# joshua16266261/self-play-ai

Hardware: AMD Instinct MI355X
Metric: MCTS sims/sec + self-play games/sec, Connect4 800 sims/move, 1/2/4/8 GPU (higher is better)
Workload: dtype bf16

## Files before the change

### include/spai.h

```cpp
#ifndef SPAI_H
#define SPAI_H

#include <stddef.h>
#include <stdint.h>

#ifdef __cplusplus
extern "C" {
#endif

#define SPAI_VERSION_MAJOR 0
#define SPAI_VERSION_MINOR 4

typedef enum spai_error {
    SPAI_OK = 0,
    SPAI_ERR_INVALID = -1,
    SPAI_ERR_ILLEGAL_MOVE = -2,
    SPAI_ERR_GAME_OVER = -3,
    SPAI_ERR_DEVICE = -4,
    SPAI_ERR_NAN = -5,
    SPAI_ERR_CAPACITY = -6,
    SPAI_ERR_UNSUPPORTED = -7
} spai_error;

typedef enum spai_game { SPAI_GAME_TICTACTOE = 0, SPAI_GAME_CONNECT4 = 1, SPAI_GAME_CHESS = 2 } spai_game;
// ... 72 lines not shown
                                 const float *policies , const float *values ,
                                 const int32_t *moves );
typedef struct spai_selfplay_stats {
    double sims;
    double evals;
    double games;
    double positions;
    double moves;
    double seconds;
} spai_selfplay_stats;
int spai_selfplay_run(spai_engine *eng, uint32_t n_games, uint64_t game_id_base, spai_sample_sink sink, void *user,
                      spai_selfplay_stats *stats);
int spai_selfplay_stream(spai_engine *eng, uint32_t n_games, uint32_t window, uint64_t game_id_base,
                         spai_sample_sink sink, void *user, spai_selfplay_stats *stats);

int spai_eval_cache_set_capacity(spai_engine *eng, uint64_t entries);
typedef struct spai_eval_cache_stats {
    double lookups;
    double hits;
    double inserts;
    double dropped;
    double clears;
    double capacity;
} spai_eval_cache_stats;
int spai_eval_cache_get_stats(spai_engine *eng, spai_eval_cache_stats *out);

typedef struct spai_match_player {
    int32_t eval;
    uint32_t num_searches;
    spai_net *net;
} spai_match_player;
typedef struct spai_match_config {
    uint32_t struct_size;
    uint32_t opening_plies;
    uint64_t seed;
} spai_match_config;
typedef struct spai_match_game {
    uint64_t game_id;
    int8_t a_moves_first;
    int8_t result_a;
    uint8_t n_moves;
    uint8_t moves[42];
} spai_match_game;
typedef struct spai_match_stats {
    double a_wins[2], draws[2], b_wins[2];
    double sims[2], evals[2];
    double seconds;
} spai_match_stats;
// ... 281 lines not shown
```

### self-play-ai_amd/csrc/capi.cpp

```cpp
#include <cstdarg>
#include <cstdio>
#include <cstring>
#include <new>

#include "philox.h"
#include "spai_internal.h"

namespace spai {
namespace {
thread_local char g_err[1024] = "";
}

void set_error(const char *fmt, ...) {
    va_list ap;
    va_start(ap, fmt);
    vsnprintf(g_err, sizeof(g_err), fmt, ap);
    va_end(ap);
}

namespace {
float philox_unit(uint64_t seed, uint32_t tensor, uint64_t idx) {
    uint32_t key[2] = {(uint32_t)seed, (uint32_t)(seed >> 32)};
    uint32_t ctr[4] = {(uint32_t)idx, (uint32_t)(idx >> 32), tensor, 0x5EEDu};
    uint32_t out[4];
// ... 284 lines not shown
        SPAI_PTR(values);
    }
    return net_predict(n, cnt, s, priors, values);
}

int spai_engine_set_net(spai_engine *e, spai_net *n) {
    ENG_CHECK(e);
    SPAI_CHECK(!n || n->eng == e, SPAI_ERR_INVALID, "net belongs to another engine");
    e->net = n;
    return eval_cache_clear(e);
}

int spai_eval_cache_set_capacity(spai_engine *e, uint64_t entries) {
    ENG_CHECK(e);
    return eval_cache_set_capacity(e, entries);
}

int spai_eval_cache_get_stats(spai_engine *e, spai_eval_cache_stats *out) {
    ENG_CHECK(e);
    SPAI_PTR(out);
    return eval_cache_stats(e, out);
}

int spai_trees_create(spai_engine *e, uint32_t n) { ENG_CHECK(e); return trees_create(e, n); }
int spai_tree_reset(spai_engine *e, uint32_t t, const spai_c4_state *root) { ENG_CHECK(e); return tree_reset(e, t, root); }
int spai_search(spai_engine *e, uint32_t n, const uint32_t *tree_idx, uint32_t num_searches, float *policy,
                uint32_t *child_ids, float *child_visits, uint32_t *n_children) {
    ENG_CHECK(e);
    if (n) SPAI_PTR(tree_idx);
    return search(e, n, tree_idx, num_searches, policy, child_ids, child_visits, n_children, nullptr);
}
int spai_tree_use_subtree(spai_engine *e, uint32_t t, uint32_t child) { ENG_CHECK(e); return tree_use_subtree(e, t, child); }
int spai_tree_node(spai_engine *e, uint32_t t, uint32_t node, spai_c4_state *st, uint32_t *visits, float *w) {
    ENG_CHECK(e);
    return tree_node(e, t, node, st, visits, w);
}
int spai_tree_child_stats(spai_engine *e, uint32_t t, uint32_t *child_ids, uint32_t *visits, float *value_sums,
                          float *priors, uint32_t *n_children) {
    ENG_CHECK(e);
    return tree_child_stats(e, t, child_ids, visits, value_sums, priors, n_children);
}
int spai_tree_size(spai_engine *e, uint32_t t, uint32_t *nodes) {
    ENG_CHECK(e);
    SPAI_PTR(nodes);
    return tree_size(e, t, nodes);
}
// ... 313 lines not shown
```

### self-play-ai_amd/csrc/search.hip

```cpp
#include <algorithm>
#include <cstdlib>
#include <cstring>

#include "search_internal.h"

namespace spai {
namespace {

constexpr int kLanesPerTree = 8;
constexpr int kBlock = 64;
constexpr int kTreesPerBlock = kBlock / kLanesPerTree;
constexpr uint32_t kErrNan = 1u, kErrCapacity = 2u, kErrDepth = 4u;

constexpr uint32_t kPriorMark = 0x80000000u;
constexpr int kGenShift = 49;

__device__ __forceinline__ float ucb(float sqrt_np, const uint4 &ch, float c) {
    const uint32_t n = ch.x;
    const float w = __uint_as_float(ch.y), prior = __uint_as_float(ch.z);
    const float qv = ((-w / (float)(n == 0 ? 1u : n)) + 1.0f) / 2.0f;
    const float q = n == 0 ? 0.0f : qv;
    float u = c * prior;
    u = u * sqrt_np;
    u = u / (1.0f + (float)n);
// ... 120 lines not shown
    }
    if (lane8 == 0) T.depth[t] = (uint8_t)d;
    if (status != c4::kOngoing) {
        backup_nodes(nodes, pr, d, c4::terminal_value(status), lane8);
        return kTerminal;
    }
    return kLive;
}

struct CacheBuckets {
    uint32_t b0, b1;
};
__device__ __forceinline__ CacheBuckets cache_buckets(const CacheView &C, uint64_t mine, uint64_t theirs) {
    const uint64_t h = c4::splitmix64(mine ^ (theirs * 0x9E3779B97F4A7C15ull));
    const uint32_t b0 = (uint32_t)(h >> 32) & C.mask, b1 = (uint32_t)h & C.mask;
    return CacheBuckets{b0, b1 == b0 ? (b0 ^ 1u) & C.mask : b1};
}
__device__ __forceinline__ uint4 *cache_way(const CacheView &C, uint32_t bucket, int way) {
    return C.tab + ((size_t)bucket * EvalCache::kWays + (uint32_t)way) * 4;
}

enum Claim { kClaimFull, kClaimDone, kClaimSame };
__device__ __forceinline__ Claim cache_claim(uint4 *bucket, uint32_t empty, uint64_t k0, uint64_t k1, const uint4 &e1,
                                             const uint4 &e2) {
    for (int w = empty ? __ffs(empty) - 1 : (int)EvalCache::kWays; w < (int)EvalCache::kWays; ++w) {
        uint4 *e = bucket + 4 * w;
        const unsigned long long old = atomicCAS((unsigned long long *)e, 0ull, (unsigned long long)k0);
        if (old == 0ull) {
            ((uint64_t *)e)[1] = k1;
            e[1] = e1;
            e[2] = e2;
            return kClaimDone;
        }
        if (old == k0) return kClaimSame;
    }
    return kClaimFull;
}

__device__ __forceinline__ bool cache_insert(const CacheView &C, const BatchView &B, uint32_t s, int lane8) {
    const uint64_t mine = B.mine[s], theirs = B.theirs[s];
    const uint64_t gen = (uint64_t)C.gen << kGenShift;
    const uint64_t k0 = mine | gen, k1 = theirs | gen;
    const CacheBuckets cb = cache_buckets(C, mine, theirs);
    uint4 *bk0 = cache_way(C, cb.b0, 0), *bk1 = cache_way(C, cb.b1, 0);
    const uint64_t seen0 = *(const uint64_t *)(bk0 + 4 * lane8);
    const uint64_t seen1 = *(const uint64_t *)(bk1 + 4 * lane8);
    const float4 pa = *(const float4 *)(B.priors + (size_t)s * kPriorStride);
    const float4 pb = *(const float4 *)(B.priors + (size_t)s * kPriorStride + 4);
    const float value = B.value[s];
    const uint32_t same = group_bits(__ballot(seen0 == k0 || seen1 == k0));
    const uint32_t empty0 = group_bits(__ballot(seen0 == 0ull));
    const uint32_t empty1 = cb.b1 != cb.b0 ? group_bits(__ballot(seen1 == 0ull)) : 0u;
    if (same || lane8 != 0) return false;
    const uint32_t p0 = __float_as_uint(pa.x), p2 = __float_as_uint(pa.z), p4 = __float_as_uint(pb.x),
                   p6 = __float_as_uint(pb.z);
    if (((p0 | p2 | p4 | p6) & kPriorMark) != 0u) return false;
    const uint4 e1 = make_uint4(p0 | kPriorMark, __float_as_uint(pa.y), p2 | kPriorMark, __float_as_uint(pa.w));
    const uint4 e2 = make_uint4(p4 | kPriorMark, __float_as_uint(pb.y), p6 | kPriorMark, __float_as_uint(value));
    const bool second = c4::popc32(empty1) > c4::popc32(empty0);
    Claim r = cache_claim(second ? bk1 : bk0, second ? empty1 : empty0, k0, k1, e1, e2);
    if (r == kClaimFull && cb.b1 != cb.b0) r = cache_claim(second ? bk0 : bk1, second ? empty0 : empty1, k0, k1, e1, e2);
    if (r == kClaimFull) atomicAdd(C.ctr + 1, 1u);
    return r == kClaimDone;
}
__device__ __forceinline__ void cache_count(const CacheView &C, bool claimed) {
    const uint64_t b = __ballot(claimed);
    if (b && (threadIdx.x & 63) == (uint32_t)__ffsll((unsigned long long)__ballot(true)) - 1u)
        atomicAdd(C.ctr, (uint32_t)c4::popc64(b));
}

__device__ __forceinline__ bool cache_holds(const uint4 &q0, const uint4 &q1, const uint4 &q2, uint64_t k0, uint64_t k1) {
    return (((uint64_t)q0.y << 32) | q0.x) == k0 && (((uint64_t)q0.w << 32) | q0.z) == k1 &&
           (q1.x & q1.z & q2.x & q2.z & kPriorMark) != 0u;
}

__device__ __forceinline__ void slot_leaf(const TreeView &T, const BatchView &B, const CacheView &C, uint32_t t,
                                          int lane8, uint64_t x, uint64_t o, uint8_t n) {
    const bool xm = c4::x_to_move(n);
    const uint64_t mine = xm ? x : o, theirs = xm ? o : x;
    if (lane8 == 0)
        __hip_atomic_fetch_add(T.evals + t, 1u, __ATOMIC_RELAXED, __HIP_MEMORY_SCOPE_AGENT);
    if (C.tab) {
        const CacheBuckets cb = cache_buckets(C, mine, theirs);
        const uint4 *ea = cache_way(C, cb.b0, lane8), *eb = cache_way(C, cb.b1, lane8);
// ... 1 lines not shown
        const uint64_t gen = (uint64_t)C.gen << kGenShift;
        const uint64_t k0 = mine | gen, k1 = theirs | gen;
        const bool match_a = cache_holds(a0, a1, a2, k0, k1), match_b = cache_holds(b0, b1, b2, k0, k1);
        const bool match = match_a || match_b;
        const uint4 q1 = match_a ? a1 : b1, q2 = match_a ? a2 : b2;
        const uint32_t hit = group_bits(__ballot(match));
        if (hit) {
            uint32_t slot = 0;
            if (lane8 == 0) {
                slot = B.cap - 1u - atomicAdd(B.hits, 1u);
                T.slot[t] = slot | kHitSlot;
                B.tree[slot] = t;
                B.mine[slot] = mine;
                B.theirs[slot] = theirs;
            }
            slot = (uint32_t)__shfl((int)slot, 0, kLanesPerTree);
            if (lane8 == __ffs(hit) - 1) {
                float4 *pr = (float4 *)(B.priors + (size_t)slot * kPriorStride);
                pr[0] = make_float4(__uint_as_float(q1.x & ~kPriorMark), __uint_as_float(q1.y),
                                    __uint_as_float(q1.z & ~kPriorMark), __uint_as_float(q1.w));
                pr[1] = make_float4(__uint_as_float(q2.x & ~kPriorMark), __uint_as_float(q2.y),
                                    __uint_as_float(q2.z & ~kPriorMark), 0.f);
                B.value[slot] = __uint_as_float(q2.w);
            }
            return;
        }
    }
    if (lane8 == 0) {
        const uint32_t slot = atomicAdd(B.count, 1u);
        T.slot[t] = slot;
        B.tree[slot] = t;
        B.mine[slot] = mine;
        B.theirs[slot] = theirs;
    }
}

template <bool RUN_ON>
__device__ __forceinline__ void select_tree(const TreeView &T, const BatchView &B, const CacheView &C, uint32_t t,
                                            RootInfo &root, int lane8, float c, uint32_t *err, uint32_t run_cap) {
    if (lane8 == 0) T.slot[t] = kNoSlot;
    uint64_t x, o;
    uint8_t n;
    if (!RUN_ON) {
        if (descend(T, t, root, lane8, c, err, x, o, n) == kLive) slot_leaf(T, B, C, t, lane8, x, o, n);
        return;
    }
// ... 130 lines not shown
        const bool claimed = fwd && cache_insert(C, B, s, lane8);
        cache_count(C, claimed);
    }
}

__global__ void k_root_stats(TreeView T, const uint32_t *__restrict__ active, uint32_t n_active, uint32_t *out,
                             uint32_t *max_evals) {
    const uint32_t i = blockIdx.x * blockDim.x + threadIdx.x;
    if (i >= n_active) return;
    const uint32_t t = active[i];
    atomicMax(max_evals, T.evals[t]);
    atomicAdd(max_evals + 1, T.evals[t]);
    const uint4 *nodes = T.nodes + (size_t)t * T.cap;
    const uint4 r = nodes[T.root[t]];
    out[i * 8] = r.w;
    const uint32_t nch = r.w == kNoChildren ? 0 : r.w >> 24, first = r.w & 0xFFFFFFu;
    for (uint32_t k = 0; k < 7; ++k) out[i * 8 + 1 + k] = k < nch ? nodes[first + k].x : 0u;
}

__global__ void k_trees_init(TreeView T, RootsOut R, uint32_t first_tree, uint32_t n) {
    const uint32_t i = blockIdx.x * blockDim.x + threadIdx.x;
    if (i < n) tree_clear(T, R, first_tree + i);
}
}

TreeView tree_view(spai_engine *e) {
    Trees &T = e->trees;
    return TreeView{T.nodes.p, T.cap, T.root.p, T.next_free.p, T.root_x.p, T.root_o.p, T.root_n.p, T.root_status.p,
                    T.path.p, T.depth.p, T.slot.p, T.left.p, T.evals.p};
}

static BatchView batch_view(spai_engine *e, int chain, uint32_t it, bool cached) {
    Batch &B = e->batch[chain];
    const size_t h = (size_t)(it & 1u) * B.cap;
    return BatchView{B.iter_counts.p + it, B.iter_more.p ? B.iter_more.p + it : nullptr, B.tree.p + h, B.mine.p + h, B.theirs.p + h,
                     B.priors.p + h * kPriorStride, B.value.p + h,
                     cached ? B.iter_hits.p + it : nullptr, B.cap};
}

CacheView cache_view(spai_engine *e) {
    EvalCache &C = e->cache;
    if (!C.buckets) return CacheView{nullptr, 0u, 0u, nullptr};
    return CacheView{C.table.p, C.buckets - 1u, C.gen, C.ctr.p};
}

int cache_clear(spai_engine *e) {
    EvalCache &C = e->cache;
    if (!C.buckets) return SPAI_OK;
    uint32_t fill = 0;
    SPAI_HIP(hipMemcpyAsync(&fill, C.ctr.p, 4, hipMemcpyDeviceToHost, e->stream));
    SPAI_HIP(hipStreamSynchronize(e->stream));
    C.inserts_cleared += fill;
    SPAI_HIP(hipMemsetAsync(C.table.p, 0, C.table.n * sizeof(uint4), e->stream));
    SPAI_HIP(hipMemsetAsync(C.ctr.p, 0, 4, e->stream));
    C.gen = C.gen % 32767u + 1u;
    C.fill_seen = 0;
    C.clears += 1;
    return SPAI_OK;
}

int cache_prepare(spai_engine *e, bool for_net) {
    EvalCache &C = e->cache;
    if (C.ready && C.for_net == for_net) return SPAI_OK;
    C.for_net = for_net;
    uint64_t want = 0;
    if (for_net) {
        const char *v = std::getenv("SPAI_EVAL_CACHE");
        if (C.user_set) want = C.requested;
        else if (v) want = std::strtoull(v, nullptr, 10);
        else {
            size_t free_bytes = 0, total_bytes = 0;
            SPAI_HIP(hipMemGetInfo(&free_bytes, &total_bytes));
            want = std::min<uint64_t>(EvalCache::kEntriesPerTree * std::max(1u, e->cfg.max_trees),
                                      total_bytes / EvalCache::kDefaultDeviceShare / EvalCache::kEntryBytes);
        }
    }
    uint32_t buckets = 0;
    if (want) {
        buckets = 1;
        while ((uint64_t)buckets * 2 * EvalCache::kWays <= want && buckets < (1u << 28)) buckets *= 2;
    }
    if (buckets != C.buckets) {
        SPAI_HIP(hipStreamSynchronize(e->stream));
        if (C.buckets) {
            uint32_t fill = 0;
            SPAI_HIP(hipMemcpy(&fill, C.ctr.p, 4, hipMemcpyDeviceToHost));
            C.inserts_cleared += fill;
        }
        C.buckets = 0;
        if (C.ctr.p) SPAI_HIP(hipMemsetAsync(C.ctr.p, 0, 4, e->stream));
        const bool by_default = !C.user_set && !std::getenv("SPAI_EVAL_CACHE");
        int rc = C.table.alloc((size_t)buckets * EvalCache::kWays * 4);
        while (rc != SPAI_OK && by_default) {
            (void)hipGetLastError();
            buckets = buckets / 2 >= EvalCache::kMinDefaultBuckets ? buckets / 2 : 0;
            rc = C.table.alloc((size_t)buckets * EvalCache::kWays * 4);
        }
        SPAI_TRY(rc);
        if (buckets) {
            if (!C.ctr.p) {
                SPAI_TRY(C.ctr.alloc(2));
                SPAI_HIP(hipMemsetAsync(C.ctr.p, 0, 8, e->stream));
            }
            C.buckets = buckets;
            SPAI_TRY(cache_clear(e));
        }
    }
    C.ready = true;
    return SPAI_OK;
}

constexpr double kMinChainLeaves = 64;
constexpr double kTailLeaves = 0.05;
constexpr uint32_t kTailTreeEvals = 160;
constexpr uint32_t kTailRun = 128;
static int env_int(const char *name, int dflt) {
    const char *v = std::getenv(name);
    return v ? std::atoi(v) : dflt;
}
struct ChainPolicy {
    int chains;
    uint32_t grid_cap;
};
static ChainPolicy chains_for(uint32_t n, double last_evals_per_iter) {
// ... 129 lines not shown
        SPAI_CHECK(!(root->x & root->o) && !((root->x | root->o) & ~c4::kBoard) && root->status <= c4::kWon,
                   SPAI_ERR_INVALID, "root is not a Connect4 bitboard");
        s = from_abi(*root);
    }
    T.h_root[t] = 0;
    T.h_root_state[t] = s;
    T.h_root_first[t] = 0;
    T.h_root_nch[t] = 0;
    k_trees_init<<<1, 64, 0, e->stream>>>(tree_view(e), roots_out(e), t, 1);
    SPAI_HIP(hipGetLastError());
    return upload_roots(e, t, 1);
}

static int evaluate(const Chain &c, hipStream_t st, const BatchView &bv, uint32_t grid_cap, int conc) {
    if (c.kind == SPAI_EVAL_NET)
        return net_eval_batch(c.net, st, bv.count, c.cnt, bv.mine, bv.theirs, bv.priors, bv.value, grid_cap, conc);
    k_eval_stub<<<(c.cnt + kBlock - 1) / kBlock, kBlock, 0, st>>>(bv, c.cnt, c.kind);
    return SPAI_OK;
}

int chains_launch(spai_engine *e, const uint32_t *trees, const Chain *chains, int nchain, uint32_t grid_cap, bool timed,
                  bool tail) {
    hipStream_t st = e->stream;
    uint32_t n = 0, iters = 0;
    int conc = 0;
    for (int h = 0; h < nchain; ++h) {
        const Chain &c = chains[h];
        if (!c.cnt) continue;
        n += c.cnt;
        iters = std::max(iters, c.iters);
        conc += c.kind == SPAI_EVAL_NET;
        Batch &B = e->batch[h];
        const uint32_t nc = std::max<uint32_t>(c.iters, 1) + (tail ? kTailChunk + 1 : 0);
        DevBuf<uint32_t> *ctr[3] = {&B.iter_counts, c.cache.tab ? &B.iter_hits : nullptr,
                                    tail ? &B.iter_more : nullptr};
        for (DevBuf<uint32_t> *b : ctr) {
            if (!b) continue;
            if (b->n < nc) SPAI_TRY(b->alloc(nc));
            SPAI_HIP(hipMemsetAsync(b->p, 0, (size_t)nc * 4, st));
        }
    }
    SPAI_HIP(hipMemcpyAsync(e->active.p, trees, (size_t)n * 4, hipMemcpyHostToDevice, st));
    SPAI_HIP(hipMemsetAsync(e->err.p, 0, 4, st));
    SPAI_HIP(hipMemsetAsync(e->trees.evals.p, 0, ((size_t)e->trees.n_trees + 2) * 4, st));
    if (n > chains[0].cnt) SPAI_HIP(hipEventRecord(e->ev_fork, st));
    for (int h = 1; h < nchain; ++h)
        if (chains[h].cnt) SPAI_HIP(hipStreamWaitEvent(e->chain_stream[h], e->ev_fork, 0));
    const TreeView tv = tree_view(e);
    timed = timed && e->timer.enabled;
    for (uint32_t it = 0; it < (tail ? 0u : iters); ++it) {
        for (int h = 0; h < nchain; ++h) {
            const Chain &c = chains[h];
            if (!c.cnt || it >= c.iters) continue;
            const hipStream_t sh = e->chain_stream[h];
            const BatchView bv = batch_view(e, h, it, c.cache.tab);
            const uint32_t nh = c.cnt, g8 = (nh + kTreesPerBlock - 1) / kTreesPerBlock;
            const uint32_t *act = e->active.p + c.off;
            const bool sample = timed && (it % e->timer.stride == 0);
            if (it == 0) {
                if (sample) SPAI_TRY(timer_record(e, 0, it, true, sh, h));
                k_select<false><<<g8, kBlock, 0, sh>>>(tv, bv, c.cache, act, nh, e->cfg.c, e->err.p, 0u);
                if (sample) SPAI_TRY(timer_record(e, 0, it, false, sh, h));
            }
            if (sample) SPAI_TRY(timer_record(e, 1, it, true, sh, h));
            SPAI_TRY(evaluate(c, sh, bv, grid_cap, std::max(conc, 1)));
            if (sample) SPAI_TRY(timer_record(e, 1, it, false, sh, h));
            if (it + 1 < c.iters) {
                const bool s2 = timed && ((it + 1) % e->timer.stride == 0);
                if (s2) SPAI_TRY(timer_record(e, 0, it + 1, true, sh, h));
                k_expand_select<false><<<g8, kBlock, 0, sh>>>(tv, bv, batch_view(e, h, it + 1, c.cache.tab), c.cache,
                                                              act, nh, e->cfg.c, e->err.p, 0u);
                if (s2) SPAI_TRY(timer_record(e, 0, it + 1, false, sh, h));
            } else {
                if (sample) SPAI_TRY(timer_record(e, 2, it, true, sh, h));
                k_expand<<<g8, kBlock, 0, sh>>>(tv, bv, c.cache, nh, e->err.p);
                if (sample) SPAI_TRY(timer_record(e, 2, it, false, sh, h));
            }
        }
    }
    SPAI_HIP(hipGetLastError());
    for (int h = 1; h < nchain; ++h) {
        if (!chains[h].cnt) continue;
        SPAI_HIP(hipEventRecord(e->ev_join[h], e->chain_stream[h]));
        SPAI_HIP(hipStreamWaitEvent(st, e->ev_join[h], 0));
    }
    return SPAI_OK;
}

int search_launch(spai_engine *e, uint32_t n, const uint32_t *tree_idx, uint32_t num_searches, SearchRun &R) {
    const int kind = (int)e->cfg.eval;
    hipStream_t st = e->stream;
    SPAI_TRY(cache_prepare(e, kind == SPAI_EVAL_NET));
    if (cache_nearly_full(e->cache)) SPAI_TRY(cache_clear(e));
    const char *tl_env = std::getenv("SPAI_TAIL_LEAVES");
    const char *tt_env = std::getenv("SPAI_TAIL_TREE_EVALS");
    const double tail_leaves = tl_env ? std::atof(tl_env) : kTailLeaves;
    const uint32_t tail_tree = tt_env ? (uint32_t)std::max(0, std::atoi(tt_env)) : kTailTreeEvals;
    const bool tail = num_searches > 0 && e->last_served_per_iter >= 0 &&
                      (e->last_served_per_iter < tail_leaves || e->last_max_tree_evals < tail_tree);
    const bool solved = e->last_served_per_iter == 0.0;
    const char *tr_env = std::getenv("SPAI_TAIL_RUN");
    const uint32_t tail_run =
        tr_env ? (uint32_t)std::max(1, std::atoi(tr_env)) : (solved ? std::max(num_searches, 1u) : kTailRun);
    const uint32_t tail_chunk = solved ? 1u : kTailChunk;
    const ChainPolicy pol = tail ? ChainPolicy{1, 0u} : chains_for(n, e->last_evals_per_iter);
    const int nchain = R.nchain = pol.chains;
    const CacheView cv = cache_view(e);
    for (int h = 0; h < nchain; ++h) {
        const uint32_t off = (uint32_t)((uint64_t)n * h / nchain);
        R.chain[h] = Chain{off, (uint32_t)((uint64_t)n * (h + 1) / nchain) - off, num_searches, kind, e->net, cv};
    }
    SPAI_TRY(chains_launch(e, tree_idx, R.chain, nchain, pol.grid_cap, true, tail));
    R.n_counts = num_searches;
    if (tail) {
        const TreeView tv = tree_view(e);
        const uint32_t g8 = (n + kTreesPerBlock - 1) / kTreesPerBlock;
        const uint32_t *act = e->active.p;
        k_set_left<<<(n + 255) / 256, 256, 0, st>>>(tv, act, n, num_searches);
        k_select<true><<<g8, kBlock, 0, st>>>(tv, batch_view(e, 0, 0, cv.tab), cv, act, n, e->cfg.c, e->err.p, tail_run);
        uint32_t p = 0, next = 1, more = 0, next_hits = 0;
        for (;;) {
            for (uint32_t q = 0; q < tail_chunk; ++q, ++p) {
                const BatchView bv = batch_view(e, 0, p, cv.tab);
                SPAI_TRY(evaluate(R.chain[0], st, bv, 0u, 1));
                k_expand_select<true><<<g8, kBlock, 0, st>>>(tv, bv, batch_view(e, 0, p + 1, cv.tab), cv, act, n,
                                                             e->cfg.c, e->err.p, tail_run);
            }
            SPAI_HIP(hipGetLastError());
            SPAI_HIP(hipMemcpyAsync(&next, e->batch[0].iter_counts.p + p, 4, hipMemcpyDeviceToHost, st));
            SPAI_HIP(hipMemcpyAsync(&more, e->batch[0].iter_more.p + p, 4, hipMemcpyDeviceToHost, st));
            if (cv.tab)
                SPAI_HIP(hipMemcpyAsync(&next_hits, e->batch[0].iter_hits.p + p, 4, hipMemcpyDeviceToHost, st));
            SPAI_HIP(hipStreamSynchronize(st));
            next += next_hits;
            if (next == 0 && more == 0) break;
// ... 154 lines not shown
        if (value_sums) memcpy(value_sums + k, &c.y, 4);
        if (priors) memcpy(priors + k, &c.z, 4);
    }
    return SPAI_OK;
}

int tree_size(spai_engine *e, uint32_t t, uint32_t *nodes) {
    Trees &T = e->trees;
    SPAI_CHECK(t < T.n_trees, SPAI_ERR_INVALID, "tree %u out of range", t);
    SPAI_HIP(hipMemcpy(nodes, T.next_free.p + t, 4, hipMemcpyDeviceToHost));
    return SPAI_OK;
}


int eval_cache_set_capacity(spai_engine *e, uint64_t entries) {
    e->cache.user_set = true;
    e->cache.requested = entries;
    e->cache.ready = false;
    return SPAI_OK;
}

int eval_cache_clear(spai_engine *e) { return cache_clear(e); }

int eval_cache_stats(spai_engine *e, spai_eval_cache_stats *out) {
    EvalCache &C = e->cache;
    uint32_t ctr[2] = {0, 0};
    SPAI_HIP(hipStreamSynchronize(e->stream));
    if (C.ctr.p) SPAI_HIP(hipMemcpy(ctr, C.ctr.p, 8, hipMemcpyDeviceToHost));
    out->lookups = C.lookups;
    out->hits = C.hits;
    out->inserts = C.inserts_cleared + ctr[0];
    out->dropped = ctr[1];
    out->clears = C.clears;
    out->capacity = (double)C.entries();
    return SPAI_OK;
}

}
```

### self-play-ai_amd/csrc/search_internal.h

```cpp
#pragma once
#include "spai_internal.h"

namespace spai {

struct TreeView {
    uint4 *nodes;
    uint32_t cap;
    const uint32_t *root;
    uint32_t *next_free;
    const uint64_t *root_x, *root_o;
    const uint8_t *root_n, *root_status;
    uint32_t *path;
    uint8_t *depth;
    uint32_t *slot;
    uint32_t *left;
    uint32_t *evals;
};
constexpr uint32_t kNoSlot = 0xFFFFFFFFu;
constexpr uint32_t kHitSlot = 0x80000000u;

struct BatchView {
    uint32_t *count;
    uint32_t *more;
    uint32_t *tree;
    uint64_t *mine, *theirs;
    float *priors;
    float *value;
    uint32_t *hits;
    uint32_t cap;
};

struct CacheView {
    uint4 *tab;
    uint32_t mask;
    uint32_t gen;
    uint32_t *ctr;
};

struct RootsOut {
    uint32_t *root;
    uint64_t *x, *o;
    uint8_t *n, *status;
};

constexpr int kMoveRec = 10;
constexpr int kRecRoot = 0, kRecVisits = 1, kRecPick = 8, kRecEvals = 9;
constexpr uint32_t kPickNone = 0x80000000u, kPickNoTable = 3u;
__host__ __device__ __forceinline__ uint32_t pick_word(int idx, int action, uint8_t status) {
    return (uint32_t)idx | (uint32_t)action << 8 | (uint32_t)status << 16;
}
inline int pick_index(uint32_t pick) { return (int)(pick & 0xFFu); }
inline int pick_action(uint32_t pick) { return (int)((pick >> 8) & 0xFFu); }
inline uint8_t pick_status(uint32_t pick) { return (uint8_t)((pick >> 16) & 0xFFu); }
inline uint32_t root_children(uint32_t children_word) { return children_word == kNoChildren ? 0 : children_word >> 24; }
inline const uint32_t *move_rec(const uint32_t *out, size_t i) { return out + 2 + i * kMoveRec; }

inline bool move_replays(const uint32_t *rec, const c4::State &rs, c4::State &cs) {
    const uint32_t pick = rec[kRecPick], legal = c4::legal_mask(rs.x, rs.o, rs.status);
    const int idx = pick_index(pick), a = pick_action(pick);
// ... 61 lines not shown

struct Chain {
    uint32_t off, cnt;
    uint32_t iters;
    int kind;
    spai_net *net;
    CacheView cache;
};
struct SearchRun {
    int nchain = 1;
    uint32_t n_counts = 0;
    Chain chain[spai_engine::kChains] = {};
};
constexpr uint32_t kTailChunk = 4;

TreeView tree_view(spai_engine *e);
CacheView cache_view(spai_engine *e);
inline RootsOut roots_out(spai_engine *e) {
    Trees &T = e->trees;
    return RootsOut{T.root.p, T.root_x.p, T.root_o.p, T.root_n.p, T.root_status.p};
}
int cache_prepare(spai_engine *e, bool for_net);
int cache_clear(spai_engine *e);
inline bool cache_nearly_full(const EvalCache &C) { return C.buckets && (uint64_t)C.fill_seen * 8 > C.entries() * 7; }
void cache_account(spai_engine *e, double served, double forwarded, uint32_t fill);
int check_device_errors(spai_engine *e, uint32_t err);
int chains_launch(spai_engine *e, const uint32_t *trees, const Chain *chains, int nchain, uint32_t grid_cap, bool timed,
                  bool tail);
int search_launch(spai_engine *e, uint32_t n, const uint32_t *tree_idx, uint32_t num_searches, SearchRun &R);
int search_finish(spai_engine *e, const SearchRun &R, uint32_t num_searches, const uint32_t *ch_counts, uint32_t err,
                  uint32_t max_tree_evals, double served, uint32_t cache_fill);
int move_buffers(spai_engine *e, size_t n_words);

struct Quiesce {
    spai_engine *e;
    uint32_t fresh_trees;
    ~Quiesce() {
        (void)hipStreamSynchronize(e->stream);
        for (hipStream_t cs : e->chain_stream)
            if (cs) (void)hipStreamSynchronize(cs);
        if (!fresh_trees) return;
        (void)cache_clear(e);
        (void)trees_create(e, fresh_trees);
    }
};

// ... 8 lines not shown
```

### self-play-ai_amd/csrc/spai_internal.h

```cpp
#pragma once
#include <hip/hip_runtime.h>
#include <stdint.h>

#include <string>
#include <vector>

#include "../../include/spai.h"
#include "c4.h"

namespace spai {

void set_error(const char *fmt, ...) __attribute__((format(printf, 1, 2)));

#define SPAI_HIP(expr)                                                                                  \
    do {                                                                                                \
        hipError_t e_ = (expr);                                                                         \
        if (e_ != hipSuccess) {                                                                         \
            ::spai::set_error("%s failed: %s (%s:%d)", #expr, hipGetErrorString(e_), __FILE__, __LINE__); \
            return SPAI_ERR_DEVICE;                                                                     \
        }                                                                                               \
    } while (0)

#define SPAI_CHECK(cond, code, ...)          \
    do {                                     \
// ... 72 lines not shown
    std::vector<uint32_t> h_root;
    std::vector<c4::State> h_root_state;
    std::vector<uint32_t> h_root_first;
    std::vector<uint8_t> h_root_nch;
};

struct Batch {
    uint32_t cap = 0;
    DevBuf<uint32_t> tree;
    DevBuf<uint64_t> mine, theirs;
    DevBuf<float> priors;
    DevBuf<float> value;
    DevBuf<uint32_t> iter_counts;
    DevBuf<uint32_t> iter_more;
    DevBuf<uint32_t> iter_hits;
};

struct EvalCache {
    static constexpr uint32_t kWays = 8;
    static constexpr uint64_t kEntriesPerTree = 16384;
    static constexpr uint64_t kEntryBytes = 64;
    static constexpr uint64_t kDefaultDeviceShare = 16;
    static constexpr uint32_t kMinDefaultBuckets = 1024;
    bool user_set = false;
    uint64_t requested = 0;
    bool ready = false;
    bool for_net = false;
    uint32_t buckets = 0;
    uint32_t gen = 0;
    DevBuf<uint4> table;
    DevBuf<uint32_t> ctr;
    uint32_t fill_seen = 0;
    double lookups = 0, hits = 0, inserts_cleared = 0, clears = 0;
    uint64_t entries() const { return (uint64_t)buckets * kWays; }
};

struct KernelTimer {
    bool enabled = false;
    uint32_t stride = 4;
    double total_ms[3] = {0, 0, 0};
    double launches[3] = {0, 0, 0};
    double items[3] = {0, 0, 0};
    std::vector<hipEvent_t> ev;
    size_t used = 0;
    std::vector<int> which;
    std::vector<uint32_t> iter;
    std::vector<int> chain;
};

}

struct spai_net {
    spai_engine *eng = nullptr;
    int blocks = 0, hidden = 0;
    int n_cu = 256;
    spai::DevBuf<uint16_t> w_stem, w_res, w_head, w_lin;
// ... 137 lines not shown
    void *user;
    spai_pipeline_event ev;
};
int replay_push(spai_replay *r, uint32_t n, const float *s, const float *p, const float *v,
                const Observer *obs = nullptr);
int replay_pop_now(spai_replay *r, uint32_t n, float *s, float *p, float *v);
int replay_size(spai_replay *r, uint32_t *n);
void choose_multiple(uint32_t n, uint32_t k, uint64_t seed, uint64_t stream, std::vector<uint32_t> &out);
int pipeline_run(const spai_pipeline_config *cfg, const float *init_params, size_t n_params, spai_pipeline_stats *st);

int trees_create(spai_engine *e, uint32_t n);
int tree_reset(spai_engine *e, uint32_t t, const spai_c4_state *root);
int search(spai_engine *e, uint32_t n, const uint32_t *tree_idx, uint32_t num_searches, float *policy,
           uint32_t *child_ids, float *child_visits, uint32_t *n_children, double *evals_out);
int tree_use_subtree(spai_engine *e, uint32_t t, uint32_t child);
int tree_node(spai_engine *e, uint32_t t, uint32_t node, spai_c4_state *st, uint32_t *visits, float *w);
int tree_child_stats(spai_engine *e, uint32_t t, uint32_t *child_ids, uint32_t *visits, float *value_sums,
                     float *priors, uint32_t *n_children);
int tree_size(spai_engine *e, uint32_t t, uint32_t *nodes);
int selfplay_run(spai_engine *e, uint32_t n_games, uint64_t gid_base, spai_sample_sink sink, void *user,
                 spai_selfplay_stats *stats, uint32_t window = 0);
int eval_cache_set_capacity(spai_engine *e, uint64_t entries);
int eval_cache_clear(spai_engine *e);
int eval_cache_stats(spai_engine *e, spai_eval_cache_stats *out);
int match_run(spai_engine *e, const spai_match_player *a, const spai_match_player *b, uint32_t n_games,
              uint64_t gid_base, const spai_match_config *cfg, spai_match_game *games, spai_match_stats *stats);

inline c4::State from_abi(const spai_c4_state &s) { return c4::State{s.x, s.o, s.num_actions_played, s.status}; }
inline spai_c4_state to_abi(const c4::State &s) {
    spai_c4_state r{};
    r.x = s.x;
    r.o = s.o;
    r.num_actions_played = s.n;
    r.status = s.status;
    return r;
}
}
```

### self-play-ai_amd/spai.py

```python
import ctypes as C
import os

import numpy as np

HERE = os.path.dirname(os.path.abspath(__file__))
LIB_PATH = os.environ.get("SPAI_LIB") or os.path.join(HERE, "libspai.so")

GAME_TICTACTOE, GAME_CONNECT4, GAME_CHESS = 0, 1, 2
EVAL_NET, EVAL_UNIFORM, EVAL_HASH = 0, 1, 2
DTYPE_BF16, DTYPE_F32 = 0, 1
ONGOING, TIED, WON = 0, 1, 2
OK = 0
ERRORS = {-1: "INVALID", -2: "ILLEGAL_MOVE", -3: "GAME_OVER", -4: "DEVICE", -5: "NAN", -6: "CAPACITY",
          -7: "UNSUPPORTED"}

SYMBOLS = [
    "spai_last_error", "spai_version", "spai_device_count", "spai_config_default", "spai_engine_create",
    "spai_engine_destroy", "spai_engine_sync", "spai_games_resize", "spai_games_reset", "spai_games_write",
    "spai_games_read", "spai_legal_mask", "spai_apply", "spai_value_terminated", "spai_encode",
    "spai_mask_invalid", "spai_rules_bench", "spai_net_num_params", "spai_net_init_params", "spai_net_create",
    "spai_net_destroy", "spai_net_forward", "spai_predict", "spai_engine_set_net", "spai_trees_create",
    "spai_tree_reset", "spai_search", "spai_tree_use_subtree", "spai_tree_node", "spai_tree_child_stats", "spai_tree_size",
    "spai_selfplay_run", "spai_selfplay_stream", "spai_eval_cache_set_capacity", "spai_eval_cache_get_stats",
    "spai_match_config_default", "spai_match_run",
    "spai_engine_set_timing", "spai_engine_timing", "spai_engine_timing_items",
    "spai_net_phase_cycles", "spai_net_bench", "spai_net_bench_conc", "spai_adam_config_default", "spai_learner_create", "spai_learner_destroy",
    "spai_learner_train_batch", "spai_learner_train_batches", "spai_learner_params", "spai_learner_grads", "spai_learner_activation", "spai_comm_unique_id",
    "spai_learner_set_comm", "spai_learner_broadcast", "spai_learner_set_host_comm", "spai_learner_last_batch",
    "spai_comm_create", "spai_comm_allreduce_f64", "spai_comm_info", "spai_comm_destroy",
    "spai_params_save_safetensors", "spai_params_load_safetensors",
    "spai_replay_create", "spai_replay_destroy", "spai_replay_push", "spai_replay_pop", "spai_replay_size",
    "spai_choose_multiple", "spai_pipeline_config_default", "spai_pipeline_run", "spai_learner_train",
    "spai_policy_normalize", "spai_policy_best_action", "spai_policy_sample",
    "spai_chess_config_default", "spai_chess_create", "spai_chess_destroy", "spai_chess_sync",
    "spai_chess_games_resize", "spai_chess_games_write", "spai_chess_games_read", "spai_chess_legal_moves",
    "spai_chess_apply", "spai_chess_status", "spai_chess_encode", "spai_chess_rules_bench", "spai_chess_perft", "spai_chess_mask_invalid",
    "spai_chess_move_index", "spai_chess_index_move", "spai_chess_net_num_params", "spai_chess_net_init_params",
    "spai_chess_net_create", "spai_chess_net_create_dtype", "spai_chess_net_dtype", "spai_chess_net_destroy", "spai_chess_net_forward", "spai_chess_predict", "spai_chess_set_net",
    "spai_chess_trees_create", "spai_chess_search", "spai_chess_tree_reset", "spai_chess_tree_use_subtree", "spai_chess_tree_root", "spai_chess_trees_advance",
    "spai_chess_selfplay_run", "spai_chess_selfplay_stream", "spai_chess_set_timing", "spai_chess_timing",
    "spai_chess_net_set_params", "spai_chess_learner_create", "spai_chess_learner_destroy",
    "spai_chess_learner_train_batch", "spai_chess_learner_train", "spai_chess_learner_params",
    "spai_chess_learner_grads", "spai_chess_learner_activation", "spai_chess_learner_last_batch",
    "spai_chess_learner_set_compute", "spai_chess_learner_get_compute", "spai_chess_learner_set_capture",
    "spai_chess_learner_gradient", "spai_chess_learner_logits",
    "spai_chess_match_config_default", "spai_chess_match_run", "spai_chess_tree_children",
# ... 12 lines not shown


class SpaiError(RuntimeError):
    def __init__(self, code, msg):
        super().__init__(f"spai error {code} ({ERRORS.get(code, '?')}): {msg}")
        self.code = code


class C4State(C.Structure):
    _fields_ = [("x", C.c_uint64), ("o", C.c_uint64), ("num_actions_played", C.c_uint8), ("status", C.c_uint8),
                ("pad", C.c_uint8 * 6)]


class Config(C.Structure):
    _fields_ = [("c", C.c_float), ("num_searches", C.c_uint32), ("temperature", C.c_float),
                ("max_trees", C.c_uint32), ("max_moves", C.c_uint32), ("eval", C.c_uint32), ("seed", C.c_uint64)]


class SelfPlayStats(C.Structure):
    _fields_ = [(k, C.c_double) for k in ("sims", "evals", "games", "positions", "moves", "seconds")]


class EvalCacheStats(C.Structure):
    _fields_ = [(k, C.c_double) for k in ("lookups", "hits", "inserts", "dropped", "clears", "capacity")]


class MatchPlayer(C.Structure):
    _fields_ = [("eval", C.c_int32), ("num_searches", C.c_uint32), ("net", C.c_void_p)]


class MatchConfig(C.Structure):
    _fields_ = [("struct_size", C.c_uint32), ("opening_plies", C.c_uint32), ("seed", C.c_uint64)]


class MatchGame(C.Structure):
    _fields_ = [("game_id", C.c_uint64), ("a_moves_first", C.c_int8), ("result_a", C.c_int8),
                ("n_moves", C.c_uint8), ("moves", C.c_uint8 * 42)]


class MatchStats(C.Structure):
    _fields_ = [(k, C.c_double * 2) for k in ("a_wins", "draws", "b_wins", "sims", "evals")] + \
               [("seconds", C.c_double)]


class AdamConfig(C.Structure):
    _fields_ = [(k, C.c_float) for k in ("lr", "beta1", "beta2", "eps", "bn_momentum", "bn_eps")]

# ... 60 lines not shown
        L.spai_apply.argtypes = [vp, u32, u32, vp, vp]
        L.spai_value_terminated.argtypes = [vp, u32, u32, vp, vp]
        L.spai_encode.argtypes = [vp, u32, u32, vp]
        L.spai_mask_invalid.argtypes = [vp, u32, u32, vp, u32, vp]
        L.spai_rules_bench.argtypes = [vp, u32, u32, vp]
        L.spai_net_num_params.argtypes = [i32, i32, i32, P(C.c_size_t)]
        L.spai_net_init_params.argtypes = [i32, i32, i32, u64, vp]
        L.spai_net_create.argtypes = [vp, i32, i32, vp, C.c_size_t, i32, P(vp)]
        L.spai_net_destroy.argtypes = [vp]
        L.spai_net_forward.argtypes = [vp, u32, vp, vp, vp]
        L.spai_predict.argtypes = [vp, u32, vp, vp, vp]
        L.spai_engine_set_net.argtypes = [vp, vp]
        L.spai_trees_create.argtypes = [vp, u32]
        L.spai_tree_reset.argtypes = [vp, u32, vp]
        L.spai_search.argtypes = [vp, u32, vp, u32, vp, vp, vp, vp]
        L.spai_tree_use_subtree.argtypes = [vp, u32, u32]
        L.spai_tree_node.argtypes = [vp, u32, u32, vp, vp, vp]
        L.spai_tree_child_stats.argtypes = [vp, u32, vp, vp, vp, vp, P(u32)]
        L.spai_tree_size.argtypes = [vp, u32, vp]
        L.spai_selfplay_run.argtypes = [vp, u32, u64, SINK, vp, P(SelfPlayStats)]
        L.spai_selfplay_stream.argtypes = [vp, u32, u32, u64, SINK, vp, P(SelfPlayStats)]
        L.spai_eval_cache_set_capacity.argtypes = [vp, u64]
        L.spai_eval_cache_get_stats.argtypes = [vp, P(EvalCacheStats)]
        L.spai_match_config_default.argtypes = [P(MatchConfig)]
        L.spai_match_run.argtypes = [vp, P(MatchPlayer), P(MatchPlayer), u32, u64, P(MatchConfig), P(MatchGame),
                                     P(MatchStats)]
        L.spai_engine_set_timing.argtypes = [vp, i32]
        L.spai_engine_timing.argtypes = [vp, vp, vp]
        L.spai_engine_timing_items.argtypes = [vp, vp, vp]
        L.spai_net_phase_cycles.argtypes = [vp, u32, vp]
        L.spai_net_bench.argtypes = [vp, u32, u32, vp]
        L.spai_net_bench_conc.argtypes = [vp, u32, u32, i32, vp]
        L.spai_adam_config_default.argtypes = [P(AdamConfig)]
        L.spai_learner_create.argtypes = [vp, i32, i32, vp, C.c_size_t, P(AdamConfig), P(vp)]
        L.spai_learner_destroy.argtypes = [vp]
        L.spai_learner_train_batch.argtypes = [vp, u32, vp, vp, vp, vp]
        L.spai_learner_train_batches.argtypes = [vp, u32, u32, vp, vp, vp, vp]
        L.spai_learner_params.argtypes = [vp, vp, C.c_size_t]
        L.spai_learner_grads.argtypes = [vp, vp, C.c_size_t]
        L.spai_learner_activation.argtypes = [vp, C.c_int, vp, C.c_size_t]
        L.spai_learner_train.argtypes = [vp, u32, vp, vp, vp, u32, u32, u64, vp]
        L.spai_comm_unique_id.argtypes = [vp]
        L.spai_learner_set_comm.argtypes = [vp, i32, i32, vp]
        L.spai_learner_broadcast.argtypes = [vp, i32]
        L.spai_learner_set_host_comm.argtypes = [vp, i32, i32, HOST_ALLREDUCE, vp]
        L.spai_learner_last_batch.argtypes = [vp, P(u32)]
# ... 252 lines not shown
            cfg.opening_plies = opening_plies
        cfg.seed = seed
        pl = []
        for kind, net, sims in (a, b):
            pl.append(MatchPlayer(int(kind), int(sims), net.h if net is not None else None))
        out = (MatchGame * max(n_games, 1))()
        st = MatchStats()
        _check(lib().spai_match_run(self.h, C.byref(pl[0]), C.byref(pl[1]), n_games, game_id_base, C.byref(cfg), out,
                                    C.byref(st)))
        games = [dict(game=int(g.game_id), a_moves_first=bool(g.a_moves_first), result_a=int(g.result_a),
                      moves=[int(m) for m in g.moves[:g.n_moves]]) for g in out[:n_games]]
        stats = {k: [float(v) for v in getattr(st, k)] for k in ("a_wins", "draws", "b_wins", "sims", "evals")}
        stats["seconds"] = float(st.seconds)
        return games, stats

    def set_eval_cache(self, entries):
        _check(lib().spai_eval_cache_set_capacity(self.h, int(entries)))

    def eval_cache_stats(self):
        st = EvalCacheStats()
        _check(lib().spai_eval_cache_get_stats(self.h, C.byref(st)))
        return {k: getattr(st, k) for k, _ in EvalCacheStats._fields_}

    def set_timing(self, on, stride=None):
        k = 1 if not stride else -1 if stride == 1 else int(stride)
        _check(lib().spai_engine_set_timing(self.h, k if on else 0))

    def timing(self):
        avg = np.zeros(3, np.float64)
        launches = np.zeros(3, np.float64)
        tot = np.zeros(3, np.float64)
        items = np.zeros(3, np.float64)
        _check(lib().spai_engine_timing(self.h, _p(avg), _p(launches)))
        _check(lib().spai_engine_timing_items(self.h, _p(tot), _p(items)))
        names = ("select", "evaluate", "expand")
        return {nm: dict(avg_ms=avg[i], launches=launches[i], total_ms=tot[i], items=items[i])
                for i, nm in enumerate(names)}


class Learner:

    def __init__(self, engine, blocks, params, hidden=64, **adam):
        cfg = AdamConfig()
        _check(lib().spai_adam_config_default(C.byref(cfg)))
        for k, v in adam.items():
            setattr(cfg, k, float(v))
# ... 216 lines not shown
```

Before: 74.12 million.

## Thin eval cache by age and hit history instead of clearing when full

When the evaluation cache nears capacity, it is now partially evicted instead of wiped. Each entry records an insert sequence number and a last-hit sequence number. A histogram kernel bins live entries by age and hit class, the host picks age cutoffs that keep about half the capacity (favouring entries that have been hit), and a sweep kernel zeroes the rest. This keeps cache hits, and so avoids repeated network evaluations, across what used to be full clears. The cost is two extra table-wide passes with a host sync, extra stores on insert and hit, and a fuller table that may drop more inserts.

```diff
diff --git a/include/spai.h b/include/spai.h
--- a/include/spai.h
+++ b/include/spai.h
@@ -118,8 +118,13 @@
     double dropped;
     double clears;
     double capacity;
+    double thins;
+    double evicted;
+    double live;
+    double kept_hit;
 } spai_eval_cache_stats;
 int spai_eval_cache_get_stats(spai_engine *eng, spai_eval_cache_stats *out);
+int spai_eval_cache_thin(spai_engine *eng, uint64_t keep_entries);
 
 typedef struct spai_match_player {
     int32_t eval;
diff --git a/self-play-ai_amd/csrc/capi.cpp b/self-play-ai_amd/csrc/capi.cpp
--- a/self-play-ai_amd/csrc/capi.cpp
+++ b/self-play-ai_amd/csrc/capi.cpp
@@ -330,6 +330,11 @@
     return eval_cache_stats(e, out);
 }
 
+int spai_eval_cache_thin(spai_engine *e, uint64_t keep_entries) {
+    ENG_CHECK(e);
+    return eval_cache_thin(e, keep_entries);
+}
+
 int spai_trees_create(spai_engine *e, uint32_t n) { ENG_CHECK(e); return trees_create(e, n); }
 int spai_tree_reset(spai_engine *e, uint32_t t, const spai_c4_state *root) { ENG_CHECK(e); return tree_reset(e, t, root); }
 int spai_search(spai_engine *e, uint32_t n, const uint32_t *tree_idx, uint32_t num_searches, float *policy,
diff --git a/self-play-ai_amd/csrc/search.hip b/self-play-ai_amd/csrc/search.hip
--- a/self-play-ai_amd/csrc/search.hip
+++ b/self-play-ai_amd/csrc/search.hip
@@ -1,4 +1,5 @@
 #include <algorithm>
+#include <cstdio>
 #include <cstdlib>
 #include <cstring>
 
@@ -166,7 +167,7 @@
 
 enum Claim { kClaimFull, kClaimDone, kClaimSame };
 __device__ __forceinline__ Claim cache_claim(uint4 *bucket, uint32_t empty, uint64_t k0, uint64_t k1, const uint4 &e1,
-                                             const uint4 &e2) {
+                                             const uint4 &e2, uint32_t seq) {
     for (int w = empty ? __ffs(empty) - 1 : (int)EvalCache::kWays; w < (int)EvalCache::kWays; ++w) {
         uint4 *e = bucket + 4 * w;
         const unsigned long long old = atomicCAS((unsigned long long *)e, 0ull, (unsigned long long)k0);
@@ -174,6 +175,7 @@
             ((uint64_t *)e)[1] = k1;
             e[1] = e1;
             e[2] = e2;
+            *(uint32_t *)(e + 3) = seq;
             return kClaimDone;
         }
         if (old == k0) return kClaimSame;
@@ -202,8 +204,9 @@
     const uint4 e1 = make_uint4(p0 | kPriorMark, __float_as_uint(pa.y), p2 | kPriorMark, __float_as_uint(pa.w));
     const uint4 e2 = make_uint4(p4 | kPriorMark, __float_as_uint(pb.y), p6 | kPriorMark, __float_as_uint(value));
     const bool second = c4::popc32(empty1) > c4::popc32(empty0);
-    Claim r = cache_claim(second ? bk1 : bk0, second ? empty1 : empty0, k0, k1, e1, e2);
-    if (r == kClaimFull && cb.b1 != cb.b0) r = cache_claim(second ? bk0 : bk1, second ? empty0 : empty1, k0, k1, e1, e2);
+    Claim r = cache_claim(second ? bk1 : bk0, second ? empty1 : empty0, k0, k1, e1, e2, C.seq);
+    if (r == kClaimFull && cb.b1 != cb.b0)
+        r = cache_claim(second ? bk0 : bk1, second ? empty0 : empty1, k0, k1, e1, e2, C.seq);
     if (r == kClaimFull) atomicAdd(C.ctr + 1, 1u);
     return r == kClaimDone;
 }
@@ -251,6 +254,7 @@
                 pr[1] = make_float4(__uint_as_float(q2.x & ~kPriorMark), __uint_as_float(q2.y),
                                     __uint_as_float(q2.z & ~kPriorMark), 0.f);
                 B.value[slot] = __uint_as_float(q2.w);
+                ((uint32_t *)((match_a ? ea : eb) + 3))[1] = C.seq;
             }
             return;
         }
@@ -427,6 +431,46 @@
     const uint32_t i = blockIdx.x * blockDim.x + threadIdx.x;
     if (i < n) tree_clear(T, R, first_tree + i);
 }
+
+struct ThinEntry {
+    bool live;
+    uint32_t cls;
+    uint32_t age;
+};
+__device__ __forceinline__ ThinEntry thin_entry(const uint4 &q, uint32_t now) {
+    const uint32_t c0 = (uint32_t)__shfl((int)q.x, 0, 4), c1 = (uint32_t)__shfl((int)q.y, 0, 4);
+    const uint32_t born = (uint32_t)__shfl((int)q.x, 3, 4), hit = (uint32_t)__shfl((int)q.y, 3, 4);
+    const uint32_t age = now - (hit ? hit : born);
+    return ThinEntry{(c0 | c1) != 0u, hit ? 1u : 0u, age < EvalCache::kAges - 1 ? age : EvalCache::kAges - 1};
+}
+
+__global__ __launch_bounds__(256) void k_thin_count(const uint4 *__restrict__ tab, size_t quarters, uint32_t now,
+                                                    uint32_t *hist) {
+    __shared__ uint32_t bins[2 * EvalCache::kAges];
+    for (uint32_t b = threadIdx.x; b < 2 * EvalCache::kAges; b += blockDim.x) bins[b] = 0u;
+    __syncthreads();
+    const size_t stride = (size_t)gridDim.x * blockDim.x;
+    for (size_t i = (size_t)blockIdx.x * blockDim.x + threadIdx.x; i < quarters; i += stride) {
+        const ThinEntry te = thin_entry(tab[i], now);
+        if ((i & 3) == 0 && te.live) atomicAdd(&bins[te.cls * EvalCache::kAges + te.age], 1u);
+    }
+    __syncthreads();
+    for (uint32_t b = threadIdx.x; b < 2 * EvalCache::kAges; b += blockDim.x)
+        if (bins[b]) atomicAdd(hist + b, bins[b]);
+}
+
+__global__ __launch_bounds__(256) void k_thin_sweep(uint4 *__restrict__ tab, size_t quarters, uint32_t now,
+                                                    uint32_t cut_fresh, uint32_t cut_hit, uint32_t *live) {
+    const size_t stride = (size_t)gridDim.x * blockDim.x;
+    uint32_t kept = 0;
+    for (size_t i = (size_t)blockIdx.x * blockDim.x + threadIdx.x; i < quarters; i += stride) {
+        const ThinEntry te = thin_entry(tab[i], now);
+        const bool drop = te.live && te.age >= (te.cls ? cut_hit : cut_fresh);
+        if (drop) tab[i] = make_uint4(0u, 0u, 0u, 0u);
+        kept += (uint32_t)c4::popc64(__ballot((i & 3) == 0 && te.live && !drop));
+    }
+    if ((threadIdx.x & 63) == 0 && kept) atomicAdd(live, kept);
+}
 }
 
 TreeView tree_view(spai_engine *e) {
@@ -445,8 +489,8 @@
 
 CacheView cache_view(spai_engine *e) {
     EvalCache &C = e->cache;
-    if (!C.buckets) return CacheView{nullptr, 0u, 0u, nullptr};
-    return CacheView{C.table.p, C.buckets - 1u, C.gen, C.ctr.p};
+    if (!C.buckets) return CacheView{nullptr, 0u, 0u, nullptr, 0u};
+    return CacheView{C.table.p, C.buckets - 1u, C.gen, C.ctr.p, C.seq};
 }
 
 int cache_clear(spai_engine *e) {
@@ -461,6 +505,72 @@
     C.gen = C.gen % 32767u + 1u;
     C.fill_seen = 0;
     C.clears += 1;
+    return SPAI_OK;
+}
+
+constexpr uint64_t kHitShareNum = 3, kHitShareDen = 4;
+struct ThinCut {
+    uint32_t cut[2];
+    uint64_t kept[2], seen[2];
+};
+static ThinCut thin_cutoff(const uint32_t *hist, uint64_t keep) {
+    ThinCut t{{0u, 0u}, {0, 0}, {0, 0}};
+    for (uint32_t cls = 0; cls < 2; ++cls)
+        for (uint32_t a = 0; a < EvalCache::kAges; ++a) t.seen[cls] += hist[cls * EvalCache::kAges + a];
+    if (t.seen[0] + t.seen[1] <= keep) {
+        t.cut[0] = t.cut[1] = EvalCache::kAges;
+        t.kept[0] = t.seen[0];
+        t.kept[1] = t.seen[1];
+        return t;
+    }
+    for (int cls = 1; cls >= 0; --cls) {
+        const uint64_t budget = cls ? keep * kHitShareNum / kHitShareDen : keep - t.kept[1];
+        const uint32_t *h = hist + cls * EvalCache::kAges;
+        while (t.cut[cls] < EvalCache::kAges && t.kept[cls] + h[t.cut[cls]] <= budget) t.kept[cls] += h[t.cut[cls]++];
+    }
+    return t;
+}
+
+uint64_t cache_keep_budget(const EvalCache &C) {
+    const char *v = std::getenv("SPAI_EVAL_CACHE_KEEP");
+    const double f = v ? std::min(1.0, std::max(0.0, std::atof(v))) : 0.5;
+    return (uint64_t)((double)C.entries() * f);
+}
+
+int cache_thin(spai_engine *e, uint64_t keep) {
+    EvalCache &C = e->cache;
+    if (!C.buckets) return SPAI_OK;
+    hipStream_t st = e->stream;
+    const size_t quarters = C.table.n;
+    int n_cu = 0;
+    SPAI_HIP(hipDeviceGetAttribute(&n_cu, hipDeviceAttributeMultiprocessorCount, e->device));
+    const uint32_t grid = (uint32_t)std::min<size_t>((quarters + 255) / 256, (size_t)std::max(1, n_cu) * 8);
+    uint32_t *hist = C.ctr.p + 2;
+    uint32_t h[2 * EvalCache::kAges];
+    SPAI_HIP(hipMemsetAsync(hist, 0, sizeof(h), st));
+    k_thin_count<<<grid, 256, 0, st>>>(C.table.p, quarters, C.seq, hist);
+    SPAI_HIP(hipGetLastError());
+    SPAI_HIP(hipMemcpyAsync(h, hist, sizeof(h), hipMemcpyDeviceToHost, st));
+    SPAI_HIP(hipStreamSynchronize(st));
+    const ThinCut t = thin_cutoff(h, keep);
+    const uint64_t seen = t.seen[0] + t.seen[1], kept = t.kept[0] + t.kept[1];
+    if (kept == seen) return SPAI_OK;
+    SPAI_HIP(hipMemsetAsync(C.ctr.p, 0, 4, st));
+    k_thin_sweep<<<grid, 256, 0, st>>>(C.table.p, quarters, C.seq, t.cut[0], t.cut[1], C.ctr.p);
+    SPAI_HIP(hipGetLastError());
+    C.inserts_cleared += (double)(seen - kept);
+    C.evicted += (double)(seen - kept);
+    C.kept_hit = (double)t.kept[1];
+    C.fill_seen = (uint32_t)kept;
+    C.thins += 1;
+    C.clears += 1;
+    const char *log = std::getenv("SPAI_EVAL_CACHE_THIN_LOG");
+    if (log && std::atoi(log))
+        std::fprintf(stderr, "eval cache thin %.0f: call %u, keep %llu of %llu live: hit %llu kept %llu (age < %u), "
+                             "never hit %llu kept %llu (age < %u)\n",
+                     C.thins, C.seq, (unsigned long long)keep, (unsigned long long)seen, (unsigned long long)t.seen[1],
+                     (unsigned long long)t.kept[1], t.cut[1], (unsigned long long)t.seen[0],
+                     (unsigned long long)t.kept[0], t.cut[0]);
     return SPAI_OK;
 }
 
@@ -504,7 +614,7 @@
         SPAI_TRY(rc);
         if (buckets) {
             if (!C.ctr.p) {
-                SPAI_TRY(C.ctr.alloc(2));
+                SPAI_TRY(C.ctr.alloc(EvalCache::kCtrWords));
                 SPAI_HIP(hipMemsetAsync(C.ctr.p, 0, 8, e->stream));
             }
             C.buckets = buckets;
@@ -680,6 +790,7 @@
 int chains_launch(spai_engine *e, const uint32_t *trees, const Chain *chains, int nchain, uint32_t grid_cap, bool timed,
                   bool tail) {
     hipStream_t st = e->stream;
+    const uint32_t seq = e->cache.seq = e->cache.seq + 1u ? e->cache.seq + 1u : 1u;
     uint32_t n = 0, iters = 0;
     int conc = 0;
     for (int h = 0; h < nchain; ++h) {
@@ -712,12 +823,14 @@
             if (!c.cnt || it >= c.iters) continue;
             const hipStream_t sh = e->chain_stream[h];
             const BatchView bv = batch_view(e, h, it, c.cache.tab);
+            CacheView cache = c.cache;
+            cache.seq = seq;
             const uint32_t nh = c.cnt, g8 = (nh + kTreesPerBlock - 1) / kTreesPerBlock;
             const uint32_t *act = e->active.p + c.off;
             const bool sample = timed && (it % e->timer.stride == 0);
             if (it == 0) {
                 if (sample) SPAI_TRY(timer_record(e, 0, it, true, sh, h));
-                k_select<false><<<g8, kBlock, 0, sh>>>(tv, bv, c.cache, act, nh, e->cfg.c, e->err.p, 0u);
+                k_select<false><<<g8, kBlock, 0, sh>>>(tv, bv, cache, act, nh, e->cfg.c, e->err.p, 0u);
                 if (sample) SPAI_TRY(timer_record(e, 0, it, false, sh, h));
             }
             if (sample) SPAI_TRY(timer_record(e, 1, it, true, sh, h));
@@ -726,12 +839,12 @@
             if (it + 1 < c.iters) {
                 const bool s2 = timed && ((it + 1) % e->timer.stride == 0);
                 if (s2) SPAI_TRY(timer_record(e, 0, it + 1, true, sh, h));
-                k_expand_select<false><<<g8, kBlock, 0, sh>>>(tv, bv, batch_view(e, h, it + 1, c.cache.tab), c.cache,
+                k_expand_select<false><<<g8, kBlock, 0, sh>>>(tv, bv, batch_view(e, h, it + 1, c.cache.tab), cache,
                                                               act, nh, e->cfg.c, e->err.p, 0u);
                 if (s2) SPAI_TRY(timer_record(e, 0, it + 1, false, sh, h));
             } else {
                 if (sample) SPAI_TRY(timer_record(e, 2, it, true, sh, h));
-                k_expand<<<g8, kBlock, 0, sh>>>(tv, bv, c.cache, nh, e->err.p);
+                k_expand<<<g8, kBlock, 0, sh>>>(tv, bv, cache, nh, e->err.p);
                 if (sample) SPAI_TRY(timer_record(e, 2, it, false, sh, h));
             }
         }
@@ -749,7 +862,7 @@
     const int kind = (int)e->cfg.eval;
     hipStream_t st = e->stream;
     SPAI_TRY(cache_prepare(e, kind == SPAI_EVAL_NET));
-    if (cache_nearly_full(e->cache)) SPAI_TRY(cache_clear(e));
+    if (cache_nearly_full(e->cache)) SPAI_TRY(cache_thin(e, cache_keep_budget(e->cache)));
     const char *tl_env = std::getenv("SPAI_TAIL_LEAVES");
     const char *tt_env = std::getenv("SPAI_TAIL_TREE_EVALS");
     const double tail_leaves = tl_env ? std::atof(tl_env) : kTailLeaves;
@@ -763,12 +876,13 @@
     const uint32_t tail_chunk = solved ? 1u : kTailChunk;
     const ChainPolicy pol = tail ? ChainPolicy{1, 0u} : chains_for(n, e->last_evals_per_iter);
     const int nchain = R.nchain = pol.chains;
-    const CacheView cv = cache_view(e);
+    CacheView cv = cache_view(e);
     for (int h = 0; h < nchain; ++h) {
         const uint32_t off = (uint32_t)((uint64_t)n * h / nchain);
         R.chain[h] = Chain{off, (uint32_t)((uint64_t)n * (h + 1) / nchain) - off, num_searches, kind, e->net, cv};
     }
     SPAI_TRY(chains_launch(e, tree_idx, R.chain, nchain, pol.grid_cap, true, tail));
+    cv.seq = e->cache.seq;
     R.n_counts = num_searches;
     if (tail) {
         const TreeView tv = tree_view(e);
@@ -969,6 +1083,8 @@
 
 int eval_cache_clear(spai_engine *e) { return cache_clear(e); }
 
+int eval_cache_thin(spai_engine *e, uint64_t keep_entries) { return cache_thin(e, keep_entries); }
+
 int eval_cache_stats(spai_engine *e, spai_eval_cache_stats *out) {
     EvalCache &C = e->cache;
     uint32_t ctr[2] = {0, 0};
@@ -980,7 +1096,11 @@
     out->dropped = ctr[1];
     out->clears = C.clears;
     out->capacity = (double)C.entries();
-    return SPAI_OK;
-}
-
-}
+    out->thins = C.thins;
+    out->evicted = C.evicted;
+    out->live = C.buckets ? (double)ctr[0] : 0.0;
+    out->kept_hit = C.kept_hit;
+    return SPAI_OK;
+}
+
+}
diff --git a/self-play-ai_amd/csrc/search_internal.h b/self-play-ai_amd/csrc/search_internal.h
--- a/self-play-ai_amd/csrc/search_internal.h
+++ b/self-play-ai_amd/csrc/search_internal.h
@@ -35,6 +35,7 @@
     uint32_t mask;
     uint32_t gen;
     uint32_t *ctr;
+    uint32_t seq;
 };
 
 struct RootsOut {
@@ -142,6 +143,8 @@
 }
 int cache_prepare(spai_engine *e, bool for_net);
 int cache_clear(spai_engine *e);
+int cache_thin(spai_engine *e, uint64_t keep_entries);
+uint64_t cache_keep_budget(const EvalCache &C);
 inline bool cache_nearly_full(const EvalCache &C) { return C.buckets && (uint64_t)C.fill_seen * 8 > C.entries() * 7; }
 void cache_account(spai_engine *e, double served, double forwarded, uint32_t fill);
 int check_device_errors(spai_engine *e, uint32_t err);
diff --git a/self-play-ai_amd/csrc/spai_internal.h b/self-play-ai_amd/csrc/spai_internal.h
--- a/self-play-ai_amd/csrc/spai_internal.h
+++ b/self-play-ai_amd/csrc/spai_internal.h
@@ -118,6 +118,8 @@
     static constexpr uint64_t kEntryBytes = 64;
     static constexpr uint64_t kDefaultDeviceShare = 16;
     static constexpr uint32_t kMinDefaultBuckets = 1024;
+    static constexpr uint32_t kAges = 256;
+    static constexpr uint32_t kCtrWords = 2 + 2 * kAges;
     bool user_set = false;
     uint64_t requested = 0;
     bool ready = false;
@@ -126,8 +128,10 @@
     uint32_t gen = 0;
     DevBuf<uint4> table;
     DevBuf<uint32_t> ctr;
+    uint32_t seq = 0;
     uint32_t fill_seen = 0;
     double lookups = 0, hits = 0, inserts_cleared = 0, clears = 0;
+    double thins = 0, evicted = 0, kept_hit = 0;
     uint64_t entries() const { return (uint64_t)buckets * kWays; }
 };
 
@@ -311,6 +315,7 @@
                  spai_selfplay_stats *stats, uint32_t window = 0);
 int eval_cache_set_capacity(spai_engine *e, uint64_t entries);
 int eval_cache_clear(spai_engine *e);
+int eval_cache_thin(spai_engine *e, uint64_t keep_entries);
 int eval_cache_stats(spai_engine *e, spai_eval_cache_stats *out);
 int match_run(spai_engine *e, const spai_match_player *a, const spai_match_player *b, uint32_t n_games,
               uint64_t gid_base, const spai_match_config *cfg, spai_match_game *games, spai_match_stats *stats);
diff --git a/self-play-ai_amd/spai.py b/self-play-ai_amd/spai.py
--- a/self-play-ai_amd/spai.py
+++ b/self-play-ai_amd/spai.py
@@ -22,6 +22,7 @@
     "spai_net_destroy", "spai_net_forward", "spai_predict", "spai_engine_set_net", "spai_trees_create",
     "spai_tree_reset", "spai_search", "spai_tree_use_subtree", "spai_tree_node", "spai_tree_child_stats", "spai_tree_size",
     "spai_selfplay_run", "spai_selfplay_stream", "spai_eval_cache_set_capacity", "spai_eval_cache_get_stats",
+    "spai_eval_cache_thin",
     "spai_match_config_default", "spai_match_run",
     "spai_engine_set_timing", "spai_engine_timing", "spai_engine_timing_items",
     "spai_net_phase_cycles", "spai_net_bench", "spai_net_bench_conc", "spai_adam_config_default", "spai_learner_create", "spai_learner_destroy",
@@ -80,7 +81,8 @@
 
 
 class EvalCacheStats(C.Structure):
-    _fields_ = [(k, C.c_double) for k in ("lookups", "hits", "inserts", "dropped", "clears", "capacity")]
+    _fields_ = [(k, C.c_double) for k in ("lookups", "hits", "inserts", "dropped", "clears", "capacity",
+                                          "thins", "evicted", "live", "kept_hit")]
 
 
 class MatchPlayer(C.Structure):
@@ -187,6 +189,7 @@
         L.spai_selfplay_stream.argtypes = [vp, u32, u32, u64, SINK, vp, P(SelfPlayStats)]
         L.spai_eval_cache_set_capacity.argtypes = [vp, u64]
         L.spai_eval_cache_get_stats.argtypes = [vp, P(EvalCacheStats)]
+        L.spai_eval_cache_thin.argtypes = [vp, u64]
         L.spai_match_config_default.argtypes = [P(MatchConfig)]
         L.spai_match_run.argtypes = [vp, P(MatchPlayer), P(MatchPlayer), u32, u64, P(MatchConfig), P(MatchGame),
                                      P(MatchStats)]
@@ -485,6 +488,9 @@
         _check(lib().spai_eval_cache_get_stats(self.h, C.byref(st)))
         return {k: getattr(st, k) for k, _ in EvalCacheStats._fields_}
 
+    def eval_cache_thin(self, keep_entries):
+        _check(lib().spai_eval_cache_thin(self.h, int(keep_entries)))
+
     def set_timing(self, on, stride=None):
         k = 1 if not stride else -1 if stride == 1 else int(stride)
         _check(lib().spai_engine_set_timing(self.h, k if on else 0))
```

Result: faster. 75.35 million (median of 6 runs) (+1.7%).
